# chenjianqu/dynamic_vins

Measured on AMD Instinct MI355X. Metric: stereo frames/sec (track+BA), higher is better.
Workload: dtype f64; 1 GPU; synthetic 1280x720 stereo @20 Hz + IMU @200 Hz, ZED intrinsics with distortion, figure-8 in a textured box room, max_cnt 250, min_dist 25, flow_back 1, 10 solver iterations, BA + marginalization on every frame; mode=raw, config=zed, parallelism=replicas x1 (independent sequences, no collective), landmarks_in_window=266, features_per_frame=250, warmup_requested=5, gpu_max_hw_queues=4, frames=resident in HBM before the timed region

## Files before the change

### dynamic_vins_amd/csrc/be_api.hip

```cpp
#include <algorithm>
#include <atomic>
#include <condition_variable>
#include <mutex>
#include "dv_ctx.h"
#include "be_kernels.h"

static_assert(sizeof(dv_ba_factor) == sizeof(BeFactor), "public/private factor layouts must match");
static_assert(sizeof(dv_ba_lm) == sizeof(BeLm), "public/private landmark layouts must match");
static_assert(sizeof(dv_ba_prior) == sizeof(BePriorHdr), "public/private prior layouts must match");

static int be_ensure(dv_ctx* ctx, int nfac) {
    BeWork& w = ctx->be;
    if (w.ready && nfac <= w.fac_cap) return 0;
    const int fac_cap = std::max(nfac, BE_MAX_LM * BE_MAX_OBS_FACTORS);
    size_t off = 0;
    auto take = [&](size_t bytes) { size_t o = off; off += (bytes + 255) / 256 * 256; return o; };
    const size_t n = BE_MAX_STATE;
    size_t o_ctl = take(sizeof(BeCtl)), o_x = take(sizeof(BeState)), o_imu = take(sizeof(BeImu) * BE_WIN), o_pr = take(sizeof(BePriorHdr)), o_i = take(4 * 4 * n),
           o_mt = take(4 * BE_MARG_TAB_INTS), o_lm = take(sizeof(BeLm) * BE_MAX_LM), o_fac = take(sizeof(BeFactor) * (size_t)fac_cap);
    const size_t upload_bytes = off;
    size_t o_c = take(sizeof(BeState)),
           o_pA = take(8 * (size_t)BE_MAX_PRIOR * BE_MAX_PRIOR), o_pb = take(8 * BE_MAX_PRIOR),
           o_pA2 = take(8 * (size_t)BE_MAX_PRIOR * BE_MAX_PRIOR), o_pb2 = take(8 * BE_MAX_PRIOR), o_ms = take(64), o_c0 = take(64),
           o_pk = take(8 * (size_t)BE_PK_SIZE * BE_PK_STRIDE), o_io = take(8 * (size_t)BE_WIN * IMU_OUT_STRIDE), o_po = take(8 * (BE_MAX_PRIOR + 1)),
           o_cc = take(8 * (BE_MAX_LM + BE_WIN + 1)), o_ob = take(4 * BE_MAX_LM), o_hd = take(8 * n * n), o_sc = take(8 * n * n), o_g = take(8 * 2 * n),
           o_pk1 = take(8 * (size_t)BE_PK_SIZE * BE_PK_STRIDE), o_io1 = take(8 * (size_t)BE_WIN * IMU_OUT_STRIDE), o_po1 = take(8 * (BE_MAX_PRIOR + 1)),
           o_hd1 = take(8 * n * n), o_sc1 = take(8 * n * n), o_g1 = take(8 * 2 * n),
           o_v = take(8 * 4 * n), o_vl = take(8 * 4 * (size_t)BE_MAX_LM);
    DV_CHECK(w.block.ensure(off));
    uint8_t* b = (uint8_t*)w.block.p;
    w.ctl = (BeCtl*)(b + o_ctl); w.x = (BeState*)(b + o_x); w.cand = (BeState*)(b + o_c); w.fac = (BeFactor*)(b + o_fac); w.lm = (BeLm*)(b + o_lm);
    w.imu = (BeImu*)(b + o_imu); w.prior = (BePriorHdr*)(b + o_pr);
    w.priorA_buf[0] = (double*)(b + o_pA); w.priorb_buf[0] = (double*)(b + o_pb); w.priorA_buf[1] = (double*)(b + o_pA2); w.priorb_buf[1] = (double*)(b + o_pb2);
    w.prior_cur = 0; w.priorA = w.priorA_buf[0]; w.priorb = w.priorb_buf[0]; w.prior_resident = false;
    w.marg_tab = (int32_t*)(b + o_mt); w.marg_scal = (double*)(b + o_ms); w.prior_c0 = (double*)(b + o_c0);
    w.packets[0] = (double*)(b + o_pk); w.imu_out[0] = (double*)(b + o_io); w.prior_out[0] = (double*)(b + o_po); w.cand_cost = (double*)(b + o_cc); w.lm_obs = (int32_t*)(b + o_ob);
    w.Hd[0] = (double*)(b + o_hd); w.Sc[0] = (double*)(b + o_sc); w.gvec[0] = (double*)(b + o_g);
    w.packets[1] = (double*)(b + o_pk1); w.imu_out[1] = (double*)(b + o_io1); w.prior_out[1] = (double*)(b + o_po1);
    w.Hd[1] = (double*)(b + o_hd1); w.Sc[1] = (double*)(b + o_sc1); w.gvec[1] = (double*)(b + o_g1);
    double* v = (double*)(b + o_v); w.scale_p = v; w.diag_p = v + n; w.grad_p = v + 2 * n; w.gn_p = v + 3 * n;
    double* vl = (double*)(b + o_vl); w.scale_l = vl; w.diag_l = vl + BE_MAX_LM; w.grad_l = vl + 2 * BE_MAX_LM; w.gn_l = vl + 3 * BE_MAX_LM;
    int32_t* iv = (int32_t*)(b + o_i); w.prior_col = iv; w.col_kind = iv + n; w.col_frame = iv + 2 * n; w.col_comp = iv + 3 * n;
    w.fac_cap = fac_cap;
    w.up_ctl = o_ctl; w.up_x = o_x; w.up_imu = o_imu; w.up_prior = o_pr; w.up_idx = o_i; w.up_mt = o_mt; w.up_lm = o_lm; w.up_fac = o_fac;
    const size_t need = upload_bytes + sizeof(BeState) + sizeof(BeCtl) + 4096;
    if (w.pinned_bytes < need) {
        if (w.pinned) (void)hipHostFree(w.pinned);
        w.pinned = nullptr;
        DV_CHECK(hipHostMalloc(&w.pinned, need, hipHostMallocDefault));
        w.pinned_bytes = need;
    }
    w.dl_off = upload_bytes;
    if (!w.ev_state) DV_CHECK(hipEventCreateWithFlags(&w.ev_state, hipEventDisableTiming));
    if (const char* e = std::getenv("DVINS_GPU_REJECT")) w.gpu_reject = std::atoi(e) != 0;
// ... 449 lines not shown
    if (ctx->dist.transport != 0) {
        const DvDist& dd = ctx->dist;
        sh.on = 1; sh.rank = dd.rank; sh.world = dd.world;
        sh.cap = std::max(1, (P->nlm + dd.world - 1) / dd.world);
        sh.lo = std::min(P->nlm, dd.rank * sh.cap); sh.hi = std::min(P->nlm, sh.lo + sh.cap);
        sh.len = BE_XS_LEN;
        sh.xsend = (double*)dd.xsend.p; sh.xrecv = (const double*)dd.xrecv.p;
        sh.qf[0] = (double*)dd.qf.p; sh.qf[1] = sh.qf[0] + BE_QF_LEN;
        ea.lm_lo = sh.lo; ea.lm_hi = sh.hi;
    }
    for (int k = 0; k < 2; ++k) { ea.packets[k] = w.packets[k]; ea.imu_out[k] = w.imu_out[k]; ea.prior_out[k] = w.prior_out[k]; }
    BeSolveArgs sa{};
    sa.ctl = w.ctl; sa.x = w.x; sa.cand = w.cand; sa.lm = w.lm; sa.imu = w.imu; sa.prior = w.prior; sa.priorA = w.priorA; sa.dims = d;
    sa.cand_cost = w.cand_cost; sa.lm_obs = w.lm_obs;
    for (int k = 0; k < 2; ++k) { sa.packets[k] = w.packets[k]; sa.imu_out[k] = w.imu_out[k]; sa.prior_out[k] = w.prior_out[k]; sa.Hd[k] = w.Hd[k]; sa.Sc[k] = w.Sc[k]; sa.gvec[k] = w.gvec[k]; }
    sa.scale_p = w.scale_p; sa.diag_p = w.diag_p; sa.grad_p = w.grad_p; sa.gn_p = w.gn_p; sa.scale_l = w.scale_l; sa.diag_l = w.diag_l; sa.grad_l = w.grad_l; sa.gn_l = w.gn_l;
    sa.prior_col = w.prior_col; sa.col_kind = w.col_kind; sa.col_frame = w.col_frame; sa.col_comp = w.col_comp;
    sa.xnorm2_extra = P->x_norm2_extra; sa.sh = sh; sa.xt = xt;
    sa.ldl_mf16 = 0;
    if (!w.ldl_generic && !(P->free_blocks & 3)) {
        uint8_t plan[64];
        if (be_mf16_plan(d.nstate, plan)) { std::memcpy(sa.ldl_col0, plan, sizeof(plan)); sa.ldl_mf16 = 1; }
    }
    pd.rej_on = false;
    if (fused && fused->want_reject && w.gpu_reject && P->nlm > 0) {
        if (!w.rej_pinned) DV_CHECK(hipHostMalloc((void**)&w.rej_pinned, BE_MAX_LM, hipHostMallocDefault));
        BeRejectArgs& r = pd.rej;
        r.st = w.cand; r.fac = w.fac; r.lm = w.lm; r.nlm = P->nlm; r.nframes = P->nframes; r.focal = fused->rej_focal; r.flags = w.rej_pinned;
        std::memcpy(r.ric, fused->rej_ric, sizeof(r.ric)); std::memcpy(r.tic, fused->rej_tic, sizeof(r.tic));
        r.ex_from_state = (P->free_blocks & 1) ? 1 : 0; r.pad = 0;
        pd.rej_on = true;
    }
    pd.xt = xt; pd.copy_ex_td = (P->free_blocks & 3) != 0;
    pd.ea = ea; pd.sa = sa; pd.fused_present = fused != nullptr; pd.fuse_accept_gauge = fused != nullptr && !ctx->batch && !sh.on ; pd.max_iters = P->max_iters; pd.g_norm = P->g_norm; pd.nframes = P->nframes; pd.use_imu = P->use_imu; pd.nlm = P->nlm;
    pd.want_raw_pose = fused && fused->want_raw_pose;
    if (fused) { std::memcpy(pd.gauge_R0, fused->R0, sizeof(pd.gauge_R0)); std::memcpy(pd.gauge_ypr0, fused->ypr0, sizeof(pd.gauge_ypr0)); std::memcpy(pd.gauge_P0, fused->P0, sizeof(pd.gauge_P0)); }
    pd.do_marg = do_marg; pd.state_bytes = state_bytes; pd.nxt = 1 - w.prior_cur;
    if (eval_only) {
        be_launch_eval(ea, BE_EVAL_X, s); be_launch_eval_ext(ea, xt, BE_EVAL_X, s);
        be_launch_reduce(sa, 0, s); be_launch_reduce_ext(sa, 0, s);
        if (sh.on) { if (be_exchange(ctx, (size_t)sh.len, s)) return -1; be_launch_shard_finalize(sa, 0, s); }
        DV_CHECK(hipGetLastError());
        return 0;
    }
    if (w.debug_hash_log && fused) {
        if (!w.dbg_pinned) DV_CHECK(hipHostMalloc((void**)&w.dbg_pinned, 64, hipHostMallocDefault));
// ... 405 lines not shown
    if (windows) *windows = B->t_windows;
    return 0;
}
int dv_batch_info(dv_batch* B, long long* batched_rounds, long long* single_rounds) {
    if (!B) return -1;
    if (batched_rounds) *batched_rounds = B->batched_rounds;
    if (single_rounds) *single_rounds = B->single_rounds;
    return 0;
}

int dv_debug_set(dv_ctx* ctx, const char* key, int value) {
    if (!ctx || !key) return -1;
    if (std::strcmp(key, "short_first_pass") == 0) { ctx->be.debug_short_first_pass = value != 0; return 0; }
    if (std::strcmp(key, "peer_timeout_ms") == 0) { ctx->dist.peer_timeout_ticks = 100000ll * std::max(value, 1); return 0; }
    if (std::strcmp(key, "batch_single_eval") == 0) { ctx->be.debug_batch_single = (ctx->be.debug_batch_single & ~1) | (value ? 1 : 0); return 0; }
    if (std::strcmp(key, "batch_single_reduce") == 0) { ctx->be.debug_batch_single = (ctx->be.debug_batch_single & ~2) | (value ? 2 : 0); return 0; }
    if (std::strcmp(key, "batch_single_tail") == 0) { ctx->be.debug_batch_single = (ctx->be.debug_batch_single & ~8) | (value ? 8 : 0); return 0; }
    if (std::strcmp(key, "batch_single_solve") == 0) { ctx->be.debug_batch_single = (ctx->be.debug_batch_single & ~4) | (value ? 4 : 0); return 0; }
    if (std::strcmp(key, "hash_light") == 0) { ctx->be.debug_hash_light = value != 0; return 0; }
    if (std::strcmp(key, "hash_log") == 0) { ctx->be.debug_hash_log = value != 0; return 0; }
    if (std::strcmp(key, "wait_tail") == 0) { ctx->be.debug_wait_tail = value != 0; return 0; }
    if (std::strcmp(key, "gpu_reject") == 0) { ctx->be.gpu_reject = value != 0; return 0; }
    if (std::strcmp(key, "c0_side") == 0) { ctx->be.c0_side = value != 0; return 0; }
    if (std::strcmp(key, "ldl_generic") == 0) { ctx->be.ldl_generic = value != 0; return 0; }
    DV_FAIL(std::string("dv_debug_set: unknown key ") + key);
}

int dv_ba_eval(dv_ctx* ctx, const dv_ba_problem* P, int* n_out, double* cost, double* S, double* g) {
    if (!ctx) return -1;
    if (!P || !n_out) DV_FAIL("dv_ba_eval: null argument");
    if (ctx->be.pend->active) DV_FAIL("dv_ba_eval: a solve is in flight");
    if (ctx->est && ctx->be.prior_resident && P->prior && P->prior->valid && P->prior_A != ctx->be.priorA_buf[ctx->be.prior_cur])
        DV_FAIL("dv_ba_eval: this ctx's estimator holds a device-resident prior; use a separate ctx for operator-level calls");
    if (be_begin_impl(ctx, const_cast<dv_ba_problem*>(P), nullptr, true)) return -1;
    BeWork& w = ctx->be;
    hipStream_t s = ctx->be_stream;
    const BePending& pd = *w.pend;
    if (pd.trivial) { w.pend->active = false; *n_out = 0; if (cost) *cost = 0; return 0; }
    const int n = pd.sa.dims.nstate, NBR = (n + 3) / 4, nblk = NBR * (NBR + 1) / 2;
    *n_out = n;
    std::vector<double> blk((size_t)nblk * 16), gv(2 * (size_t)n), lcost((size_t)std::max(P->nlm, 1)), io((size_t)std::max(P->nimu, 1) * IMU_OUT_STRIDE), pc(1);
    DV_CHECK(hipMemcpyAsync(blk.data(), w.Sc[0], 8 * blk.size(), hipMemcpyDeviceToHost, s));
    DV_CHECK(hipMemcpyAsync(gv.data(), w.gvec[0], 8 * gv.size(), hipMemcpyDeviceToHost, s));
    if (P->nlm) DV_CHECK(hipMemcpyAsync(lcost.data(), w.packets[0] + (size_t)BE_PK_COST * BE_PK_STRIDE, 8 * (size_t)P->nlm, hipMemcpyDeviceToHost, s));
    if (P->nimu) DV_CHECK(hipMemcpyAsync(io.data(), w.imu_out[0], 8 * (size_t)P->nimu * IMU_OUT_STRIDE, hipMemcpyDeviceToHost, s));
    DV_CHECK(hipMemcpyAsync(pc.data(), w.prior_out[0], 8, hipMemcpyDeviceToHost, s));
// ... 127 lines not shown
```

### dynamic_vins_amd/csrc/be_kernels.h

```cpp
#pragma once
#include <cstddef>
#include <hip/hip_runtime.h>
#include "be_factor_dev.h"

#define IMU_OUT_STRIDE 936

#define BE_XS_MSZ (66 * 36)
#define BE_XS_M(k) ((k) * BE_XS_MSZ)
#define BE_XS_V(k) (5 * BE_XS_MSZ + (k) * 66)
#define BE_XS_A (5 * BE_XS_MSZ + 8 * 66)
#define BE_XS_LEN (BE_XS_A + 16)
#define BE_XS_BUF ((BE_XS_LEN > BE_MAX_LM + 16 ? BE_XS_LEN : BE_MAX_LM + 16))
#define BE_QF_M(k) ((k) * 4356)
#define BE_QF_V(k) (4 * 4356 + (k) * 66)
#define BE_QF_A (4 * 4356 + 7 * 66)
#define BE_QF_LEN (BE_QF_A + 16)
struct BeShard { int32_t on, rank, world, lo, hi, cap, len, pad; double* xsend; const double* xrecv; double* qf[2]; };

#define BE_NX 13
#define BX_W 0
#define BX_G 13
#define BX_XX 26
#define BX_XP 195
#define BX_SIZE 1056
// ... 6 lines not shown
    BeDims dims; double g_norm;
    double* packets[2];
    double* imu_out[2];
    double* prior_out[2];
    double* cand_cost;
    int32_t* lm_obs;
    int32_t lm_lo, lm_hi;
    const double* prior_c0;
};

struct BeSolveArgs {
    BeCtl* ctl;
    BeState* x; BeState* cand;
    const BeLm* lm; const BeImu* imu; const BePriorHdr* prior; const double* priorA;
    BeDims dims;
    const double* packets[2]; const double* imu_out[2]; const double* prior_out[2]; const double* cand_cost; const int32_t* lm_obs;
    double* Hd[2];
    double* Sc[2];
    double* gvec[2];
    double* scale_p; double* diag_p; double* grad_p; double* gn_p;
    double* scale_l; double* diag_l; double* grad_l; double* gn_l;
    int32_t* prior_col;
    int32_t* col_kind; int32_t* col_frame; int32_t* col_comp;
    uint8_t ldl_col0[64]; int32_t ldl_mf16, ldl_pad;
    BeShard sh;
    double xnorm2_extra;
    BeExt xt;
};

struct BeMargArgs {
    const BeState* x; int nframes, nlm, nimu;
    const BeFactor* fac; const BeLm* lm; const BeImu* imu;
    const BePriorHdr* prior; const double* priorA; const double* priorb;
    const int32_t* prior_map;
    const int32_t* imu_map;
    const int32_t* dim_slot;
    const int32_t* dim_comp;
    int D, m; double g_norm;
    double* outA; double* outb; double* out_scalars;
    double* W; double* part; double* psum;
    int pose_dim[BE_NF], ex_dim[2], td_dim;
    int c0_mode;
    double* sum; double* lm_h; int anchor;
    double* imu_w;
    double* c0_out;
    const int32_t* lm_sel;
    uint8_t mf_plan[64]; int32_t mf16, mf_n;
};

struct BeGaugeArgs {
// ... 7 lines not shown
#if defined(__HIPCC__)
#include "wave_dpp.h"
using namespace be;
__device__ inline void be_frame_geom_dev(const BeState* s, int nframes, FrameGeom* fg, m33* ric, d3* tic, int lane) {
    if (lane < nframes) { fg[lane].R = qR(Q4(s->pose[lane])); fg[lane].P = P3(s->pose[lane]); }
    if (lane >= 32 && lane < 34) { ric[lane - 32] = qR(Q4(s->ex[lane - 32])); tic[lane - 32] = P3(s->ex[lane - 32]); }
}

__device__ inline void be_prior_dx_dev(const BePriorHdr* p, const BeState* s, double* dx, int lane, int nthreads) {
    for (int b = lane; b < p->nblocks; b += nthreads) {
        const BePriorBlock pb = p->blocks[b];
        const double* x0 = p->x0[b];
        if (pb.type == 0 || pb.type == 2) {
            const double* x = pb.type == 0 ? s->pose[pb.idx] : s->ex[pb.idx];
            for (int k = 0; k < 3; ++k) dx[pb.off + k] = x[k] - x0[k];
            const quat dq = qmul(qinv(Q4(x0)), Q4(x));
            d3 v = qvec(dq) * 2.0;
            if (!(dq.w >= 0)) v = -v;
            dx[pb.off + 3] = v.x; dx[pb.off + 4] = v.y; dx[pb.off + 5] = v.z;
        } else if (pb.type == 1) {
            for (int k = 0; k < 9; ++k) dx[pb.off + k] = s->sb[pb.idx][k] - x0[k];
        } else dx[pb.off] = s->td - x0[0];
    }
}

__device__ __forceinline__ void be_accept_body(const BeSolveArgs& a) {
    BeCtl* ctl = a.ctl;
    const BeCtl c = *ctl;
    __shared__ double red[4];
    __shared__ int s_accept;
    const int tid = threadIdx.x;
    __syncthreads();
    if (c.done || !c.pending) return;
    if (tid == 0) { ctl->slots = c.slots + 1; ctl->pending = 0; s_accept = 0; }
    const int iter = c.iter + 1;
    const int ncost = a.dims.nlm + a.dims.nimu + 1;
    double part = 0;
    {
        double cv[4];
#pragma unroll
        for (int u = 0; u < 4; ++u) cv[u] = a.cand_cost[tid + 256 * u < ncost ? tid + 256 * u : 0];
#pragma unroll
        for (int u = 0; u < 4; ++u) if (tid + 256 * u < ncost) part += cv[u];
    }
    part = wave_sum_f64(part);
    if ((tid & 63) == 0) red[tid >> 6] = part;
// ... 81 lines not shown
```

### dynamic_vins_amd/csrc/be_solve.hip

```cpp
#include <hip/hip_runtime.h>
#include <cfloat>
#include <algorithm>
#include <cstring>
#include <cstdlib>
#include "be_kernels.h"
#include "dev_once.h"
#include "wave_dpp.h"
#include "be_mf16.h"

using namespace be;

#ifdef BE_RED_TS
__device__ long long be_red_ts[64];
#define RTS(k) do { if (threadIdx.x == 0) be_red_ts[k] = wall_clock64(); } while (0)
extern "C" int dv_debug_red_ts(long long* out) { return hipMemcpyFromSymbol(out, HIP_SYMBOL(be_red_ts), sizeof(long long) * 64) == hipSuccess ? 0 : -1; }
#else
#define RTS(k) do {} while (0)
#endif
#define RED_THREADS 448
#define RED_PAIRS (BE_NF * (BE_NF + 1) / 2)
__device__ const unsigned char RED_PAIR_TAB[RED_PAIRS] = {
    150, 152, 51, 132, 98, 166, 170, 112, 147, 85, 68, 65, 32, 168, 49, 167, 118, 153, 66, 129, 96, 130, 165, 144, 33, 148, 67, 48, 102, 162, 161, 0, 97,
    133, 50, 16, 101, 134, 17, 119, 99, 84, 114, 64, 80, 100, 163, 160, 145, 149, 115, 131, 82, 164, 81, 151, 113, 117, 116, 128, 34, 136, 83, 169, 146, 135 };
__device__ __forceinline__ void red_pair(int bx, int& fi, int& fj) { const int t = RED_PAIR_TAB[bx]; fi = t >> 4; fj = t & 15; }
// ... 271 lines not shown
            if (threadIdx.x < 11 || threadIdx.x == 12) for (int w = 0; w < RED_THREADS / 64; ++w) v += s_red[w][threadIdx.x];
            else if (threadIdx.x == 11) for (int w = 0; w < RED_THREADS / 64; ++w) v = fmax(v, s_red[w][11]);
            a.sh.xsend[BE_XS_A + threadIdx.x] = v;
        }
        return;
    }
    if (eb == 0 && c.first && !SHARD)
        for (int l = threadIdx.x; l < nlm; l += RED_THREADS) a.scale_l[l] = 1.0 / (1.0 + sqrt(BE_PK(pk, BE_PK_H, l)));
    const int t = eb * RED_THREADS + threadIdx.x;
    if (t < n * n) {
        const int i = t / n, j = t - i * n;
        if (a.col_kind[i] == 0 && a.col_kind[j] == 0) return;
        const double hd = red_dense_h(a, rc, imu_out, i, j);
        Hd[t] = hd;
        if ((j >> 2) <= (i >> 2)) Sc[blk_pos(i, j, (n + 3) >> 2)] = hd;
    } else if (t < n * n + n) {
        const int i = t - n * n;
        if (a.col_kind[i] == 0) return;
        gvec[i] = red_dense_g(a, rc, imu_out, prior_out, i); gvec[n + i] = 0.0;
    }
    if (bx == RED_PAIRS + 3) RTS(9);
}

__global__ __launch_bounds__(RED_THREADS) void be_reduce_kernel(BeSolveArgs a, int spec) { be_reduce_body<false>(a, spec, blockIdx.x); }
__global__ __launch_bounds__(RED_THREADS) void be_reduce_shard_kernel(BeSolveArgs a, int spec) { be_reduce_body<true>(a, spec, blockIdx.x); }
__global__ __launch_bounds__(RED_THREADS) void be_reduce_batch_kernel(const BeSolveArgs* __restrict__ tab, int spec) {
    const DV_CONSTANT BeSolveArgs& a = *reinterpret_cast<const DV_CONSTANT BeSolveArgs*>(reinterpret_cast<uintptr_t>(tab + blockIdx.y));
    const int n = a.dims.nstate;
    if ((int)blockIdx.x >= RED_PAIRS + (n * n + n + RED_THREADS - 1) / RED_THREADS) return;
    be_reduce_body<false>(a, spec, blockIdx.x);
}
__global__ __launch_bounds__(RED_THREADS) __attribute__((amdgpu_waves_per_eu(6, 8))) void be_reduce_batch_occ_kernel(const BeSolveArgs* __restrict__ tab, int spec) {
    const DV_CONSTANT BeSolveArgs& a = *reinterpret_cast<const DV_CONSTANT BeSolveArgs*>(reinterpret_cast<uintptr_t>(tab + blockIdx.y));
    const int n = a.dims.nstate;
    if ((int)blockIdx.x >= RED_PAIRS + (n * n + n + RED_THREADS - 1) / RED_THREADS) return;
    be_reduce_body<false>(a, spec, blockIdx.x);
}
void be_launch_reduce_batch(const BeSolveArgs* tab_dev, int n_win, int max_n, int spec, hipStream_t s) {
    static const int occ_env = [] { const char* e = std::getenv("DVINS_REDUCE_OCC"); return e ? (e[0] != '0' ? 1 : 0) : -1; }();
    const bool occ = occ_env < 0 ? n_win >= 12 : occ_env != 0;
    const dim3 grid((RED_PAIRS + (max_n * max_n + max_n + RED_THREADS - 1) / RED_THREADS + 7) & ~7, n_win);
    if (occ) hipLaunchKernelGGL(be_reduce_batch_occ_kernel, grid, dim3(RED_THREADS), 0, s, tab_dev, spec);
    else hipLaunchKernelGGL(be_reduce_batch_kernel, grid, dim3(RED_THREADS), 0, s, tab_dev, spec);
}
void be_launch_reduce(const BeSolveArgs& a, int spec, hipStream_t s) {
    const int n = a.dims.nstate;
    const int total = n * n + n;
    if (a.sh.on) hipLaunchKernelGGL(be_reduce_shard_kernel, dim3(RED_PAIRS + (total + RED_THREADS - 1) / RED_THREADS + 1), dim3(RED_THREADS), 0, s, a, spec);
    else hipLaunchKernelGGL(be_reduce_kernel, dim3(RED_PAIRS + (total + RED_THREADS - 1) / RED_THREADS), dim3(RED_THREADS), 0, s, a, spec);
}

#define FIN_THREADS 256
__global__ __launch_bounds__(FIN_THREADS) void be_shard_finalize_kernel(BeSolveArgs a, int spec) {
    const BeCtl c = *a.ctl;
    if (c.done) return;
    int set = c.cur;
    if (spec && c.pending) set ^= 1;
    else if (!c.need_eval && !c.chol_fail) return;
    const int n = a.dims.nstate, W = a.sh.world, len = a.sh.len, t = threadIdx.x;
    const double* xr = a.sh.xrecv;
    double* qf = a.sh.qf[set];
    auto rsum = [&](int e) { double v = 0.0; for (int r = 0; r < W; ++r) v += xr[(size_t)r * len + e]; return v; };
    if (blockIdx.x < RED_PAIRS) {
        int fi, fj; red_pair(blockIdx.x, fi, fj);
        const bool in_win = fi < a.dims.nframes && fj < a.dims.nframes;
        const int ci0 = in_win ? a.dims.pose_col[fi] : -1, cj0 = in_win ? a.dims.pose_col[fj] : -1;
        const bool valid = ci0 >= 0 && cj0 >= 0;
        if (t < 36) {
            const int ci = t / 6, q = t - ci * 6, e = blockIdx.x * 36 + t, i66 = fi * 6 + ci, j66 = fj * 6 + q;
            const double v0 = valid ? rsum(BE_XS_M(0) + e) : 0.0, v2 = valid ? rsum(BE_XS_M(2) + e) : 0.0, v3 = valid ? rsum(BE_XS_M(3) + e) : 0.0, v4 = valid ? rsum(BE_XS_M(4) + e) : 0.0;
            qf[BE_QF_M(0) + i66 * 66 + j66] = v0; qf[BE_QF_M(1) + i66 * 66 + j66] = v2; qf[BE_QF_M(2) + i66 * 66 + j66] = v3; qf[BE_QF_M(3) + i66 * 66 + j66] = v4;
            if (fi != fj) { qf[BE_QF_M(0) + j66 * 66 + i66] = v0; qf[BE_QF_M(1) + j66 * 66 + i66] = v2; qf[BE_QF_M(2) + j66 * 66 + i66] = v3; qf[BE_QF_M(3) + j66 * 66 + i66] = v4; }
// ... 570 lines not shown
        if (k - R >= kend) bs_ld<SEG, R>(Lm, k - R, lane, cb);
        __builtin_amdgcn_sched_barrier(0);
        bs_ap<SEG, R>(ca, k, lane, x0, x1, x2);
        __builtin_amdgcn_sched_barrier(0);
        if (k - R >= kend) {
            if (k - 2 * R >= kend) bs_ld<SEG, R>(Lm, k - 2 * R, lane, ca);
            __builtin_amdgcn_sched_barrier(0);
            bs_ap<SEG, R>(cb, k - R, lane, x0, x1, x2);
            __builtin_amdgcn_sched_barrier(0);
        }
    }
    return 64 * SEG - 1;
}
template <int ROWS>
__device__ __forceinline__ void bs_rows(const double* Lm, int kt, int lane, double& x0, double& x1, double& x2) {
    const int seg = kt >> 6;
    if (seg == 0) bs_chunk<0, ROWS>(Lm, kt, lane, x0, x1, x2);
    else if (seg == 1) bs_chunk<1, ROWS>(Lm, kt, lane, x0, x1, x2);
    else bs_chunk<2, ROWS>(Lm, kt, lane, x0, x1, x2);
}

template <int NSLOT, bool MF16>
__global__ __launch_bounds__(SOL_THREADS) void be_solve_kernel(BeSolveArgs a, int spec) {
    constexpr bool SHARD = false;
#include "be_solve_body.inc"
}
template <int NSLOT, bool MF16>
__global__ __launch_bounds__(SOL_THREADS) void be_solve_batch_kernel(const BeSolveArgs* __restrict__ tab, int spec) {
    const BeSolveArgs& a = tab[blockIdx.x];
    constexpr bool SHARD = false;
#include "be_solve_body.inc"
}
__global__ __launch_bounds__(SOL_THREADS) void be_solve_shard_kernel(BeSolveArgs a, int spec) {
    constexpr int NSLOT = 1; constexpr bool MF16 = true, SHARD = true;
#include "be_solve_body.inc"
}

static size_t solve_smem(int n) {
    const size_t tri = (size_t)n * (n + 1) / 2;
    return (tri + 9 * (size_t)n + 72 + 80 + 8 + 1536) * sizeof(double);
}
static size_t solve_smem_mf16(int n) {
    const size_t NB = ((size_t)n + 16) >> 4, nt = NB * (NB + 1) / 2;
    return (std::max<size_t>(nt * 256, 3072) + 9 * (size_t)n + 72 + 80 + 8 + 1024 + 3 * 16 * NB) * sizeof(double);
}
bool be_mf16_plan(int n, uint8_t* plan , bool check_solve_lds) {
    const int NB = (n + 16) >> 4, W = SOL_THREADS / 64;
    if (NB > MF_MAXNB || (check_solve_lds && solve_smem_mf16(n) > 160 * 1024 - 512)) return false;
    int load[SOL_THREADS / 64] = { 0 };
    std::memset(plan, 0xFF, (size_t)W * 4);
    for (int j = 1; j < NB; ++j) plan[j * 4 + load[j]++] = (uint8_t)((j << 4) | (j - 1));
    for (int J = 0; J < NB - 1; ++J) {
        int el[SOL_THREADS / 64], ne = 0;
        for (int w = 0; w < W; ++w) if ((w == 0 || w >= NB || J < w) && w != J + 1 && load[w] < 4) el[ne++] = w;
        auto key = [&](int w) { return ((1 <= w && w < NB) ? w - 1 : NB) * 1024 + load[w] * 32 + w; };
        std::sort(el, el + ne, [&](int x, int y) { return key(x) < key(y); });
        if (ne < NB - 2 - J) return false;
// ... 44 lines not shown
```

### dynamic_vins_amd/csrc/be_solve_body.inc

```
    extern __shared__ __attribute__((aligned(16))) double sm[];
    BeCtl* ctl = a.ctl;
    BeCtl c = *ctl;
    const int n = a.dims.nstate, nlm = a.dims.nlm, tid = threadIdx.x;
    const int lm0 = SHARD ? a.sh.lo : 0, nown = SHARD ? a.sh.hi - a.sh.lo : nlm;
    if (c.done) return;
    __shared__ int s_pcol[BE_NF], s_scol[BE_NF];
    if (tid < BE_NF) { s_pcol[tid] = tid < a.dims.nframes ? a.dims.pose_col[tid] : -1; s_scol[tid] = tid < a.dims.nframes ? a.dims.sb_col[tid] : -1; }
    __shared__ int s_xcol[MF16 ? 1 : 16]; __shared__ double qx[MF16 ? 1 : 16];
    bool xt_on = false;
    if constexpr (!MF16) { xt_on = a.xt.on != 0; if (tid >= 64 && tid < 80) s_xcol[tid - 64] = (xt_on && tid - 64 < BE_NX) ? a.xt.xcol[tid - 64] : -1; }
    TS(15);
    const int cur_spec = (spec && c.pending) ? (c.cur ^ 1) : c.cur;
    double dec_cv[4] = { 0.0, 0.0, 0.0, 0.0 };
    if (MF16 && spec && c.pending && tid < 256) {
        const int ncost0 = nlm + a.dims.nimu + 1;
#pragma unroll
        for (int u = 0; u < 4; ++u) dec_cv[u] = a.cand_cost[tid + 256 * u < ncost0 ? tid + 256 * u : 0];
    }
    mf_d4 mfU[MF_SLOTS];
    double pre_h = 0.0, pre_g0 = 0.0, pre_g1 = 0.0, pre_s = 0.0;
    if (MF16 && !(c.reuse && !(spec && c.pending))) {
        mf_prefetch(a.Sc[cur_spec], reinterpret_cast<const uint8_t*>(a.ldl_col0), n, mfU);
        if (tid < n) { pre_h = a.Hd[cur_spec][(size_t)tid * n + tid]; pre_g0 = a.gvec[cur_spec][tid]; pre_g1 = a.gvec[cur_spec][n + tid]; pre_s = a.scale_p[tid]; }
    }
    if (spec && c.pending) {
        __shared__ double red4[4];
        const int ncost = nlm + a.dims.nimu + 1;
        double part = 0;
        if (tid < 256) {
            double cv[4];
#pragma unroll
            for (int u = 0; u < 4; ++u) cv[u] = MF16 ? dec_cv[u] : a.cand_cost[tid + 256 * u < ncost ? tid + 256 * u : 0];
#pragma unroll
            for (int u = 0; u < 4; ++u) if (tid + 256 * u < ncost) part += cv[u];
        }
        part = wave_sum_f64(part);
        if (tid < 256 && (tid & 63) == 0) red4[tid >> 6] = part;
        lds_barrier();
        const double cand_cost = red4[0] + red4[1] + red4[2] + red4[3];
        c.slots += 1; c.iter += 1; c.cand_cost = cand_cost; c.invalid = 0; c.pending = 0;
        bool done = false, accept = false; int term = 0;
        if (c.step_norm <= 1e-8 * (c.x_norm + 1e-8)) { done = true; term = 1; }
        else if (fabs(c.x_cost - cand_cost) <= 1e-6 * c.x_cost) { done = true; term = 1; }
        else {
            const double rel = (c.x_cost - cand_cost) / c.model_cost_change;
            if (rel > 1e-3) {
                accept = true;
                double radius = c.radius;
                if (rel < 0.25) radius *= 0.5;
                if (rel > 0.75) radius = fmax(radius, 3.0 * c.dogleg_norm);
                c.radius = radius; c.mu = fmax(1e-8, 2.0 * c.mu / 10.0);
                c.x_cost = cand_cost; c.successful += 1; c.reuse = 0; c.need_eval = 0; c.cur ^= 1;
            } else {
                c.radius = c.radius * 0.5; c.reuse = 1; c.need_eval = 0;
                if (c.radius < 1e-32) { done = true; term = 1; }
            }
            if (!done && c.iter >= c.max_iters) { done = true; term = 0; }
        }
        if (accept) {
            double* dst = reinterpret_cast<double*>(a.x);
            const double* src = reinterpret_cast<const double*>(a.cand);
            const int used = (int)(offsetof(BeState, inv_depth) / sizeof(double)) + nlm;
            for (int k = tid; k < used; k += SOL_THREADS) dst[k] = src[k];
        }
        if (done) { c.done = 1; c.termination = term; }
        if (tid == 0) *ctl = c;
        if (done) return;
        lds_barrier();
    }
    const int mf_nb = (n + 16) >> 4;
    const int npk = MF16 ? (mf_nb * (mf_nb + 1) / 2 * 256 > 3072 ? mf_nb * (mf_nb + 1) / 2 * 256 : 3072) : n * (n + 1) / 2;
    double* Lm = sm;
    double* v_s = Lm + npk;
    double* v_d = v_s + n;
    double* v_grad = v_d + n;
    double* v_gn = v_grad + n;
    double* v_t = v_gn + n;
    double* v_t2 = v_t + n;
    double* v_x = v_t2 + n;
    double* zfin = v_x + n;
    double* dvec = zfin + n;
    double* q66 = dvec + n;
    double* red = q66 + 72;
    double* misc = red + 80;
    double* scratch = MF16 ? Lm : misc + 8;
    MfLds mf; mf.Tl = Lm; mf.gat = misc + 8; mf.dv = mf.gat + 1024; mf.iv = mf.dv + 16 * mf_nb; mf.yv = mf.iv + 16 * mf_nb;
    double* PL = scratch, *PD = scratch + 4 * 184;
    double* dinfo = red;
    __shared__ int s_fail;
    const double mu = c.mu;
// ... 73 lines not shown
        if (warm_up) {
        double warm = 0.0;
        const int lpr = (nlm + 15) >> 4;
        for (int e = t; e < 66 * lpr; e += nt) { const int q = e / lpr, l16 = e - q * lpr; warm += __builtin_nontemporal_load(&BE_PK(pk, BE_PK_W + q, l16 * 16)); }
        for (int e = t; e < (n * n + 15) >> 4; e += nt) warm += __builtin_nontemporal_load(Hd + (size_t)e * 16);
        const int nst = ((int)(offsetof(BeState, inv_depth) / sizeof(double)) + nlm + 15) >> 4;
        for (int e = t; e < nst; e += nt) warm += __builtin_nontemporal_load(reinterpret_cast<const double*>(a.x) + (size_t)e * 16);
        if (warm == 1.2345e-300) misc[6] = warm;
        }
    };
    if (!c.reuse) {
        for (int i = tid; i < n; i += SOL_THREADS) {
            const bool pre = MF16 && cur_spec == c.cur;
            const double hii = pre ? pre_h : Hd[(size_t)i * n + i];
            const double s = c.first ? 1.0 / (1.0 + sqrt(hii)) : (pre ? pre_s : a.scale_p[i]);
            double d2 = hii * s * s; d2 = fmin(fmax(d2, 1e-6), 1e32);
            const double d = sqrt(d2);
            const double g0 = pre ? pre_g0 : gvec[i];
            v_s[i] = s; v_d[i] = d; v_grad[i] = g0 * s / d;
            v_x[i] = g0 - (pre ? pre_g1 : gvec[n + i]);
            if (!MF16) { if (c.first) a.scale_p[i] = s; a.diag_p[i] = d; a.grad_p[i] = v_grad[i]; }
        }
        lds_barrier();
        auto cost_and_tolerance = [&]() -> bool {
            if (c.first) {
                double part = 0;
                if (!SHARD) for (int l = tid; l < nlm; l += SOL_THREADS) part += BE_PK(pk, BE_PK_COST, l);
                for (int k = tid; k < a.dims.nimu; k += SOL_THREADS) part += imu_out[(size_t)k * IMU_OUT_STRIDE];
                if (tid == 0) part += prior_out[0];
                if (SHARD && tid == 0) part += qfc[BE_QF_A + 10];
                const double xc = block_sum(part, red);
                if (tid == 0) { ctl->x_cost = xc; ctl->initial_cost = xc; }
            }
            {
                double gm = 0;
                for (int i = tid; i < n; i += SOL_THREADS) gm = fmax(gm, fabs(gvec[i]));
                if (!SHARD) for (int l = tid; l < nlm; l += SOL_THREADS) gm = fmax(gm, fabs(BE_PK(pk, BE_PK_G, l)));
                else if (tid == 0) gm = fmax(gm, qfc[BE_QF_A + 11]);
    #pragma unroll
                for (int o = 32; o > 0; o >>= 1) gm = fmax(gm, __shfl_xor(gm, o));
                __syncthreads();
                if ((tid & 63) == 0) red[tid >> 6] = gm;
                __syncthreads();
                gm = 0; for (int k = 0; k < SOL_THREADS / 64; ++k) gm = fmax(gm, red[k]);
                __syncthreads();
                if (gm <= 1e-10) { if (tid == 0) { ctl->done = 1; ctl->termination = 1; ctl->first = 0; } return true; }
// ... 48 lines not shown
            for (int k = 0; k < SOL_THREADS / 64; ++k) { gm = fmax(gm, red[k]); xc += red[16 + k]; }
            if (c.first && tid == 0) { ctl->x_cost = xc; ctl->initial_cost = xc; }
            if (gm <= 1e-10) { if (tid == 0) { ctl->done = 1; ctl->termination = 1; ctl->first = 0; } return; }
        }
        TS(24);
        if (MF16) for (int i = tid; i < n; i += SOL_THREADS) { if (c.first) a.scale_p[i] = v_s[i]; a.diag_p[i] = v_d[i]; a.grad_p[i] = v_grad[i]; }
        TS(7);
        for (int i = tid; i < n; i += SOL_THREADS) { v_gn[i] = -v_d[i] * v_x[i]; a.gn_p[i] = v_gn[i]; v_t[i] = v_s[i] * v_x[i]; }
        lds_barrier();
        gather66(v_t);
        wdot_all();
        if (lm_live) {
            const double rho = 1.0 / (lm_h + mu * lm_diag * lm_diag / (lm_scale * lm_scale));
            lm_wgn = wd[tid];
            const double yl = rho / lm_scale * (lm_g - lm_wgn);
            lm_gn = -lm_diag * yl;
            a.gn_l[lmi] = lm_gn;
        }
        lds_barrier();
    } else {
        for (int i = tid; i < n; i += SOL_THREADS) { v_s[i] = a.scale_p[i]; v_d[i] = a.diag_p[i]; v_grad[i] = a.grad_p[i]; v_gn[i] = a.gn_p[i]; }
        if (lm_live) { lm_h = BE_PK(pk, BE_PK_H, lmi); lm_g = BE_PK(pk, BE_PK_G, lmi); lm_scale = a.scale_l[lmi]; lm_diag = a.diag_l[lmi]; lm_grad = a.grad_l[lmi]; lm_gn = a.gn_l[lmi]; }
        __syncthreads();
    }
    TS(8);
    double p_gg = 0, p_nn = 0, p_gn = 0;
    for (int i = tid; i < n; i += SOL_THREADS) { p_gg += v_grad[i] * v_grad[i]; p_nn += v_gn[i] * v_gn[i]; p_gn += v_grad[i] * v_gn[i]; }
    if (!SHARD && lm_live) { p_gg += lm_grad * lm_grad; p_nn += lm_gn * lm_gn; p_gn += lm_grad * lm_gn; }
    double f_Q2 = 0, f_Q6 = 0, f_Q9 = 0, f_L2 = 0, f_LGS = 0, f_L5 = 0, f_L6 = 0, f_L8 = 0, f_L9 = 0;
    __shared__ double vq[SHARD ? 72 : 1];
    if (SHARD) {
        if (tid < 66) { const int fa = tid / 6, r = tid - fa * 6; const int col = s_pcol[fa]; vq[tid] = col >= 0 ? -(v_s[col + r] / v_d[col + r]) * v_gn[col + r] : 0.0; }
        lds_barrier();
        double q2 = 0, q6 = 0, q9 = 0;
        for (int e = tid; e < 4356; e += SOL_THREADS) { const int i = e / 66, j = e - i * 66; const double vv = vq[i] * vq[j]; q2 += qfc[BE_QF_M(1) + e] * vv; q6 += qfc[BE_QF_M(2) + e] * vv; q9 += qfc[BE_QF_M(3) + e] * vv; }
        double l5[5] = { q2, q6, q9, 0, 0 }, l4[4] = { 0, 0, 0, 0 };
        if (tid < 66) { const double v = vq[tid]; l5[3] = v * qfc[BE_QF_V(1) + tid]; l5[4] = v * qfc[BE_QF_V(0) + tid]; l4[0] = v * qfc[BE_QF_V(3) + tid]; l4[1] = v * qfc[BE_QF_V(4) + tid]; l4[2] = v * qfc[BE_QF_V(5) + tid]; l4[3] = v * qfc[BE_QF_V(6) + tid]; }
        block_sum_n_dpp<5>(l5, red);
        block_sum_n_dpp<4>(l4, red);
        f_Q2 = l5[0]; f_Q6 = l5[1]; f_Q9 = l5[2]; f_L2 = l5[3]; f_LGS = l5[4]; f_L5 = l4[0]; f_L6 = l4[1]; f_L8 = l4[2]; f_L9 = l4[3];
        if (tid == 0) {
            const double* A = qfc + BE_QF_A;
            p_gg += A[0]; p_nn += (A[1] - 2.0 * f_L2) + f_Q2; p_gn += f_LGS - A[2];
        }
    }
    double sv3[3] = {p_gg, p_nn, p_gn};
// ... 189 lines not shown
```

### dynamic_vins_amd/csrc/dv_ctx.h

```cpp
#pragma once
#include "dv_internal.h"
#include "be_types.h"
#include "be_kernels.h"
#include <cmath>
#include <cstring>
#include <chrono>
#include <deque>
#include <map>
#include <memory>
#include <mutex>
#include <string>
#include <vector>

struct DevBuf {
    void* p = nullptr; size_t bytes = 0;
    hipError_t ensure(size_t n) {
        if (n <= bytes) return hipSuccess;
        if (p) (void)hipFree(p);
        p = nullptr; bytes = 0;
        hipError_t e = hipMalloc(&p, n);
        if (e == hipSuccess) bytes = n;
        return e;
    }
    void release() { if (p) (void)hipFree(p); p = nullptr; bytes = 0; }
// ... 42 lines not shown
struct MargPlan {
    int mode = -1, D = 0, m = 0, n = 0, nimu = 0, nsel = 0;
    bool empty = false;
    int pose_dim[BE_NF], sb_dim[BE_NF], ex_dim[2], td_dim;
    int32_t tab[BE_MARG_TAB_INTS];
};

struct BePending {
    bool want_raw_pose = false;
    bool deferred = false; int first_slots = 0;
    bool rej_on = false; BeRejectArgs rej{};
    hipEvent_t ev_state_ext = nullptr;
    bool fuse_accept_gauge = false;
    bool active = false, trivial = false, do_marg = false, fused_present = false, marg_in_flight = false, marg_check_due = false; int scal_slot = 0, check_slot = 0; size_t state_bytes = 0; int nxt = 0; MargPlan pl;
    BeExt xt{}; bool copy_ex_td = false;
    BeEvalArgs ea; BeSolveArgs sa; int max_iters = 0, nframes = 0, use_imu = 0, nlm = 0; double g_norm = 0, gauge_R0[9], gauge_ypr0[3], gauge_P0[3];
    std::chrono::steady_clock::time_point t_begin, t_up, t_enq;
};

struct BeWork {
    std::unique_ptr<BePending> pend = std::make_unique<BePending>();
    bool ready = false;
    DevBuf block;
    BeCtl* ctl = nullptr; BeState* x = nullptr; BeState* cand = nullptr;
    BeFactor* fac = nullptr; BeLm* lm = nullptr; BeImu* imu = nullptr; BePriorHdr* prior = nullptr; double* priorA = nullptr; double* priorb = nullptr;
    double* packets[2] = { nullptr, nullptr }; double* imu_out[2] = { nullptr, nullptr }; double* prior_out[2] = { nullptr, nullptr }; double* cand_cost = nullptr; int32_t* lm_obs = nullptr;
    double* Hd[2] = { nullptr, nullptr }; double* Sc[2] = { nullptr, nullptr }; double* gvec[2] = { nullptr, nullptr };
    double* scale_p = nullptr; double* diag_p = nullptr; double* grad_p = nullptr; double* gn_p = nullptr;
    double* scale_l = nullptr; double* diag_l = nullptr; double* grad_l = nullptr; double* gn_l = nullptr;
    int32_t* prior_col = nullptr; int32_t* col_kind = nullptr; int32_t* col_frame = nullptr; int32_t* col_comp = nullptr;
    int fac_cap = 0;
    DevBuf marg_buf;
    DevBuf xpk_buf;
    void* pinned = nullptr; size_t pinned_bytes = 0;
    size_t up_ctl = 0, up_x = 0, up_imu = 0, up_prior = 0, up_idx = 0, up_mt = 0, up_lm = 0, up_fac = 0, dl_off = 0;
    double* priorA_buf[2] = { nullptr, nullptr }; double* priorb_buf[2] = { nullptr, nullptr }; int prior_cur = 0;
    bool prior_resident = false;
    hipEvent_t ev_state = nullptr;
    hipStream_t c0_stream = nullptr; hipEvent_t ev_margA = nullptr, ev_c0 = nullptr; bool c0_side = false, c0_pending = false;
    double* prior_c0 = nullptr;
    int marg_form = 0;
    DevBuf eig_spec; bool eig_ran = false;
    int32_t* marg_tab = nullptr; double* marg_scal = nullptr;
    long long marg_checked = 0; double marg_last[4] = { 0, 0, 0, 0 };
    long long marg_clamped = 0;
    bool debug_short_first_pass = false, ldl_generic = false, debug_wait_tail = false; int debug_batch_single = 0; bool debug_hash_log = false, debug_hash_light = false;
    std::vector<unsigned long long> dbg_dev_log; unsigned long long* dbg_pinned = nullptr; unsigned long long dbg_solve_no = 0;
    static constexpr int DBG_RANGES = 16, DBG_SLOTS = 16;
    unsigned long long* dbg_slots = nullptr; std::vector<unsigned long long> dbg_slot_log;
    bool gpu_reject = true; uint8_t* rej_pinned = nullptr;
    std::vector<const double*> sqrt_hint;
};

bool be_imu_sqrt_info(const double* cov15x15, double* U15x15);

struct BeFused {
    int marg_mode = -1;
    double R0[9], ypr0[3], P0[3];
    dv_ba_prior new_prior;
    double diag[4] = { 0, 0, 0, 0 };
    bool want_raw_pose = false;
    bool want_reject = false; double rej_ric[2][9], rej_tic[2][3], rej_focal = 0; const uint8_t* rej_flags = nullptr;
    double raw_pose[77];
};
int be_solve_fused(dv_ctx* ctx, dv_ba_problem* P, dv_ba_summary* summary, BeFused* fused);
void be_batch_detach(dv_ctx* ctx);
struct DvFrontBatch;
DvFrontBatch*& be_batch_front(struct dv_batch* B);
int be_batch_index(struct dv_batch* B);
// ... 106 lines not shown
```

Measured before the change: 1206 frames/s.

## Move speculative accept/reject decision into an extra reduce-kernel block

Adds one extra block to the reduce kernel. In the speculative single-context MF16 path it sums the candidate costs, runs the trust-region accept/reject decision, copies the accepted candidate state into x, and writes the resulting control record to a separate ctl_dec buffer. The solve kernel then adopts that precomputed control record instead of doing the cost reduction, decision and state copy at its start. It writes the record back to ctl after its first barriers, which moves serial work off the solve kernel's critical path. This adds an extra buffer and a second control copy, with some risk of ordering subtlety between the reduce block's writes to x and other blocks.

```diff
diff --git a/dynamic_vins_amd/csrc/be_api.hip b/dynamic_vins_amd/csrc/be_api.hip
--- a/dynamic_vins_amd/csrc/be_api.hip
+++ b/dynamic_vins_amd/csrc/be_api.hip
@@ -26,10 +26,10 @@
            o_cc = take(8 * (BE_MAX_LM + BE_WIN + 1)), o_ob = take(4 * BE_MAX_LM), o_hd = take(8 * n * n), o_sc = take(8 * n * n), o_g = take(8 * 2 * n),
            o_pk1 = take(8 * (size_t)BE_PK_SIZE * BE_PK_STRIDE), o_io1 = take(8 * (size_t)BE_WIN * IMU_OUT_STRIDE), o_po1 = take(8 * (BE_MAX_PRIOR + 1)),
            o_hd1 = take(8 * n * n), o_sc1 = take(8 * n * n), o_g1 = take(8 * 2 * n),
-           o_v = take(8 * 4 * n), o_vl = take(8 * 4 * (size_t)BE_MAX_LM);
+           o_v = take(8 * 4 * n), o_vl = take(8 * 4 * (size_t)BE_MAX_LM), o_cd = take(sizeof(BeCtl));
     DV_CHECK(w.block.ensure(off));
     uint8_t* b = (uint8_t*)w.block.p;
-    w.ctl = (BeCtl*)(b + o_ctl); w.x = (BeState*)(b + o_x); w.cand = (BeState*)(b + o_c); w.fac = (BeFactor*)(b + o_fac); w.lm = (BeLm*)(b + o_lm);
+    w.ctl = (BeCtl*)(b + o_ctl); w.ctl_dec = (BeCtl*)(b + o_cd); w.x = (BeState*)(b + o_x); w.cand = (BeState*)(b + o_c); w.fac = (BeFactor*)(b + o_fac); w.lm = (BeLm*)(b + o_lm);
     w.imu = (BeImu*)(b + o_imu); w.prior = (BePriorHdr*)(b + o_pr);
     w.priorA_buf[0] = (double*)(b + o_pA); w.priorb_buf[0] = (double*)(b + o_pb); w.priorA_buf[1] = (double*)(b + o_pA2); w.priorb_buf[1] = (double*)(b + o_pb2);
     w.prior_cur = 0; w.priorA = w.priorA_buf[0]; w.priorb = w.priorb_buf[0]; w.prior_resident = false;
@@ -525,6 +525,8 @@
         uint8_t plan[64];
         if (be_mf16_plan(d.nstate, plan)) { std::memcpy(sa.ldl_col0, plan, sizeof(plan)); sa.ldl_mf16 = 1; }
     }
+    sa.ctl_dec = w.ctl_dec;
+    sa.dec_reduce = (sa.ldl_mf16 && !sh.on && !ctx->batch && !w.debug_decide_in_solve) ? 1 : 0;
     pd.rej_on = false;
     if (fused && fused->want_reject && w.gpu_reject && P->nlm > 0) {
         if (!w.rej_pinned) DV_CHECK(hipHostMalloc((void**)&w.rej_pinned, BE_MAX_LM, hipHostMallocDefault));
@@ -976,6 +978,7 @@
     if (std::strcmp(key, "wait_tail") == 0) { ctx->be.debug_wait_tail = value != 0; return 0; }
     if (std::strcmp(key, "gpu_reject") == 0) { ctx->be.gpu_reject = value != 0; return 0; }
     if (std::strcmp(key, "c0_side") == 0) { ctx->be.c0_side = value != 0; return 0; }
+    if (std::strcmp(key, "decide_in_solve") == 0) { ctx->be.debug_decide_in_solve = value != 0; return 0; }
     if (std::strcmp(key, "ldl_generic") == 0) { ctx->be.ldl_generic = value != 0; return 0; }
     DV_FAIL(std::string("dv_debug_set: unknown key ") + key);
 }
diff --git a/dynamic_vins_amd/csrc/be_kernels.h b/dynamic_vins_amd/csrc/be_kernels.h
--- a/dynamic_vins_amd/csrc/be_kernels.h
+++ b/dynamic_vins_amd/csrc/be_kernels.h
@@ -52,10 +52,11 @@
     double* scale_l; double* diag_l; double* grad_l; double* gn_l;
     int32_t* prior_col;
     int32_t* col_kind; int32_t* col_frame; int32_t* col_comp;
-    uint8_t ldl_col0[64]; int32_t ldl_mf16, ldl_pad;
+    uint8_t ldl_col0[64]; int32_t ldl_mf16, dec_reduce;
     BeShard sh;
     double xnorm2_extra;
     BeExt xt;
+    BeCtl* ctl_dec;
 };
 
 struct BeMargArgs {
@@ -109,6 +110,30 @@
             for (int k = 0; k < 9; ++k) dx[pb.off + k] = s->sb[pb.idx][k] - x0[k];
         } else dx[pb.off] = s->td - x0[0];
     }
+}
+
+__device__ __forceinline__ bool be_decide_spec(BeCtl& c, double cand_cost) {
+    c.slots += 1; c.iter += 1; c.cand_cost = cand_cost; c.invalid = 0; c.pending = 0;
+    bool done = false, accept = false; int term = 0;
+    if (c.step_norm <= 1e-8 * (c.x_norm + 1e-8)) { done = true; term = 1; }
+    else if (fabs(c.x_cost - cand_cost) <= 1e-6 * c.x_cost) { done = true; term = 1; }
+    else {
+        const double rel = (c.x_cost - cand_cost) / c.model_cost_change;
+        if (rel > 1e-3) {
+            accept = true;
+            double radius = c.radius;
+            if (rel < 0.25) radius *= 0.5;
+            if (rel > 0.75) radius = fmax(radius, 3.0 * c.dogleg_norm);
+            c.radius = radius; c.mu = fmax(1e-8, 2.0 * c.mu / 10.0);
+            c.x_cost = cand_cost; c.successful += 1; c.reuse = 0; c.need_eval = 0; c.cur ^= 1;
+        } else {
+            c.radius = c.radius * 0.5; c.reuse = 1; c.need_eval = 0;
+            if (c.radius < 1e-32) { done = true; term = 1; }
+        }
+        if (!done && c.iter >= c.max_iters) { done = true; term = 0; }
+    }
+    if (done) { c.done = 1; c.termination = term; }
+    return accept;
 }
 
 __device__ __forceinline__ void be_accept_body(const BeSolveArgs& a) {
diff --git a/dynamic_vins_amd/csrc/be_solve.hip b/dynamic_vins_amd/csrc/be_solve.hip
--- a/dynamic_vins_amd/csrc/be_solve.hip
+++ b/dynamic_vins_amd/csrc/be_solve.hip
@@ -317,7 +317,35 @@
     if (bx == RED_PAIRS + 3) RTS(9);
 }
 
-__global__ __launch_bounds__(RED_THREADS) void be_reduce_kernel(BeSolveArgs a, int spec) { be_reduce_body<false>(a, spec, blockIdx.x); }
+__device__ __forceinline__ void be_reduce_decide(const BeSolveArgs& a) {
+    BeCtl c = *a.ctl;
+    if (c.done || !c.pending) return;
+    __shared__ double red4[4];
+    const int tid = threadIdx.x, nlm = a.dims.nlm, ncost = nlm + a.dims.nimu + 1;
+    double part = 0;
+    if (tid < 256) {
+        double cv[4];
+#pragma unroll
+        for (int u = 0; u < 4; ++u) cv[u] = a.cand_cost[tid + 256 * u < ncost ? tid + 256 * u : 0];
+#pragma unroll
+        for (int u = 0; u < 4; ++u) if (tid + 256 * u < ncost) part += cv[u];
+    }
+    part = wave_sum_f64(part);
+    if (tid < 256 && (tid & 63) == 0) red4[tid >> 6] = part;
+    __syncthreads();
+    const double cand_cost = red4[0] + red4[1] + red4[2] + red4[3];
+    if (be_decide_spec(c, cand_cost)) {
+        double* dst = reinterpret_cast<double*>(a.x);
+        const double* src = reinterpret_cast<const double*>(a.cand);
+        const int used = (int)(offsetof(BeState, inv_depth) / sizeof(double)) + nlm;
+        for (int k = tid; k < used; k += RED_THREADS) dst[k] = src[k];
+    }
+    if (tid == 0) *a.ctl_dec = c;
+}
+__global__ __launch_bounds__(RED_THREADS) void be_reduce_kernel(BeSolveArgs a, int spec) {
+    if (a.dec_reduce && spec && blockIdx.x + 1 == gridDim.x) { be_reduce_decide(a); return; }
+    be_reduce_body<false>(a, spec, blockIdx.x);
+}
 __global__ __launch_bounds__(RED_THREADS) void be_reduce_shard_kernel(BeSolveArgs a, int spec) { be_reduce_body<true>(a, spec, blockIdx.x); }
 __global__ __launch_bounds__(RED_THREADS) void be_reduce_batch_kernel(const BeSolveArgs* __restrict__ tab, int spec) {
     const DV_CONSTANT BeSolveArgs& a = *reinterpret_cast<const DV_CONSTANT BeSolveArgs*>(reinterpret_cast<uintptr_t>(tab + blockIdx.y));
@@ -342,7 +370,7 @@
     const int n = a.dims.nstate;
     const int total = n * n + n;
     if (a.sh.on) hipLaunchKernelGGL(be_reduce_shard_kernel, dim3(RED_PAIRS + (total + RED_THREADS - 1) / RED_THREADS + 1), dim3(RED_THREADS), 0, s, a, spec);
-    else hipLaunchKernelGGL(be_reduce_kernel, dim3(RED_PAIRS + (total + RED_THREADS - 1) / RED_THREADS), dim3(RED_THREADS), 0, s, a, spec);
+    else hipLaunchKernelGGL(be_reduce_kernel, dim3(RED_PAIRS + (total + RED_THREADS - 1) / RED_THREADS + ((a.dec_reduce && spec) ? 1 : 0)), dim3(RED_THREADS), 0, s, a, spec);
 }
 
 #define FIN_THREADS 256
@@ -959,17 +987,17 @@
 
 template <int NSLOT, bool MF16>
 __global__ __launch_bounds__(SOL_THREADS) void be_solve_kernel(BeSolveArgs a, int spec) {
-    constexpr bool SHARD = false;
+    constexpr bool SHARD = false, DEC_RED = MF16;
 #include "be_solve_body.inc"
 }
 template <int NSLOT, bool MF16>
 __global__ __launch_bounds__(SOL_THREADS) void be_solve_batch_kernel(const BeSolveArgs* __restrict__ tab, int spec) {
     const BeSolveArgs& a = tab[blockIdx.x];
-    constexpr bool SHARD = false;
+    constexpr bool SHARD = false, DEC_RED = false;
 #include "be_solve_body.inc"
 }
 __global__ __launch_bounds__(SOL_THREADS) void be_solve_shard_kernel(BeSolveArgs a, int spec) {
-    constexpr int NSLOT = 1; constexpr bool MF16 = true, SHARD = true;
+    constexpr int NSLOT = 1; constexpr bool MF16 = true, SHARD = true, DEC_RED = false;
 #include "be_solve_body.inc"
 }
 
diff --git a/dynamic_vins_amd/csrc/be_solve_body.inc b/dynamic_vins_amd/csrc/be_solve_body.inc
--- a/dynamic_vins_amd/csrc/be_solve_body.inc
+++ b/dynamic_vins_amd/csrc/be_solve_body.inc
@@ -1,6 +1,8 @@
     extern __shared__ __attribute__((aligned(16))) double sm[];
     BeCtl* ctl = a.ctl;
     BeCtl c = *ctl;
+    const bool dec_red = DEC_RED && a.dec_reduce != 0;
+    const BeCtl cdec = *(dec_red ? a.ctl_dec : ctl);
     const int n = a.dims.nstate, nlm = a.dims.nlm, tid = threadIdx.x;
     const int lm0 = SHARD ? a.sh.lo : 0, nown = SHARD ? a.sh.hi - a.sh.lo : nlm;
     if (c.done) return;
@@ -12,7 +14,7 @@
     TS(15);
     const int cur_spec = (spec && c.pending) ? (c.cur ^ 1) : c.cur;
     double dec_cv[4] = { 0.0, 0.0, 0.0, 0.0 };
-    if (MF16 && spec && c.pending && tid < 256) {
+    if (MF16 && spec && c.pending && !dec_red && tid < 256) {
         const int ncost0 = nlm + a.dims.nimu + 1;
 #pragma unroll
         for (int u = 0; u < 4; ++u) dec_cv[u] = a.cand_cost[tid + 256 * u < ncost0 ? tid + 256 * u : 0];
@@ -23,7 +25,12 @@
         mf_prefetch(a.Sc[cur_spec], reinterpret_cast<const uint8_t*>(a.ldl_col0), n, mfU);
         if (tid < n) { pre_h = a.Hd[cur_spec][(size_t)tid * n + tid]; pre_g0 = a.gvec[cur_spec][tid]; pre_g1 = a.gvec[cur_spec][n + tid]; pre_s = a.scale_p[tid]; }
     }
-    if (spec && c.pending) {
+    bool adopt_store = false;
+    if (spec && c.pending && dec_red) {
+        c = cdec;
+        if (c.done) { if (tid == 0) *ctl = c; return; }
+        adopt_store = tid == 0;
+    } else if (spec && c.pending) {
         __shared__ double red4[4];
         const int ncost = nlm + a.dims.nimu + 1;
         double part = 0;
@@ -38,34 +45,15 @@
         if (tid < 256 && (tid & 63) == 0) red4[tid >> 6] = part;
         lds_barrier();
         const double cand_cost = red4[0] + red4[1] + red4[2] + red4[3];
-        c.slots += 1; c.iter += 1; c.cand_cost = cand_cost; c.invalid = 0; c.pending = 0;
-        bool done = false, accept = false; int term = 0;
-        if (c.step_norm <= 1e-8 * (c.x_norm + 1e-8)) { done = true; term = 1; }
-        else if (fabs(c.x_cost - cand_cost) <= 1e-6 * c.x_cost) { done = true; term = 1; }
-        else {
-            const double rel = (c.x_cost - cand_cost) / c.model_cost_change;
-            if (rel > 1e-3) {
-                accept = true;
-                double radius = c.radius;
-                if (rel < 0.25) radius *= 0.5;
-                if (rel > 0.75) radius = fmax(radius, 3.0 * c.dogleg_norm);
-                c.radius = radius; c.mu = fmax(1e-8, 2.0 * c.mu / 10.0);
-                c.x_cost = cand_cost; c.successful += 1; c.reuse = 0; c.need_eval = 0; c.cur ^= 1;
-            } else {
-                c.radius = c.radius * 0.5; c.reuse = 1; c.need_eval = 0;
-                if (c.radius < 1e-32) { done = true; term = 1; }
-            }
-            if (!done && c.iter >= c.max_iters) { done = true; term = 0; }
-        }
+        const bool accept = be_decide_spec(c, cand_cost);
         if (accept) {
             double* dst = reinterpret_cast<double*>(a.x);
             const double* src = reinterpret_cast<const double*>(a.cand);
             const int used = (int)(offsetof(BeState, inv_depth) / sizeof(double)) + nlm;
             for (int k = tid; k < used; k += SOL_THREADS) dst[k] = src[k];
         }
-        if (done) { c.done = 1; c.termination = term; }
         if (tid == 0) *ctl = c;
-        if (done) return;
+        if (c.done) return;
         lds_barrier();
     }
     const int mf_nb = (n + 16) >> 4;
@@ -185,6 +173,7 @@
             if (!MF16) { if (c.first) a.scale_p[i] = s; a.diag_p[i] = d; a.grad_p[i] = v_grad[i]; }
         }
         lds_barrier();
+        if (adopt_store) *ctl = c;
         auto cost_and_tolerance = [&]() -> bool {
             if (c.first) {
                 double part = 0;
@@ -279,6 +268,7 @@
         for (int i = tid; i < n; i += SOL_THREADS) { v_s[i] = a.scale_p[i]; v_d[i] = a.diag_p[i]; v_grad[i] = a.grad_p[i]; v_gn[i] = a.gn_p[i]; }
         if (lm_live) { lm_h = BE_PK(pk, BE_PK_H, lmi); lm_g = BE_PK(pk, BE_PK_G, lmi); lm_scale = a.scale_l[lmi]; lm_diag = a.diag_l[lmi]; lm_grad = a.grad_l[lmi]; lm_gn = a.gn_l[lmi]; }
         __syncthreads();
+        if (adopt_store) *ctl = c;
     }
     TS(8);
     double p_gg = 0, p_nn = 0, p_gn = 0;
diff --git a/dynamic_vins_amd/csrc/dv_ctx.h b/dynamic_vins_amd/csrc/dv_ctx.h
--- a/dynamic_vins_amd/csrc/dv_ctx.h
+++ b/dynamic_vins_amd/csrc/dv_ctx.h
@@ -88,7 +88,7 @@
     std::unique_ptr<BePending> pend = std::make_unique<BePending>();
     bool ready = false;
     DevBuf block;
-    BeCtl* ctl = nullptr; BeState* x = nullptr; BeState* cand = nullptr;
+    BeCtl* ctl = nullptr; BeCtl* ctl_dec = nullptr ; BeState* x = nullptr; BeState* cand = nullptr;
     BeFactor* fac = nullptr; BeLm* lm = nullptr; BeImu* imu = nullptr; BePriorHdr* prior = nullptr; double* priorA = nullptr; double* priorb = nullptr;
     double* packets[2] = { nullptr, nullptr }; double* imu_out[2] = { nullptr, nullptr }; double* prior_out[2] = { nullptr, nullptr }; double* cand_cost = nullptr; int32_t* lm_obs = nullptr;
     double* Hd[2] = { nullptr, nullptr }; double* Sc[2] = { nullptr, nullptr }; double* gvec[2] = { nullptr, nullptr };
@@ -110,7 +110,7 @@
     int32_t* marg_tab = nullptr; double* marg_scal = nullptr;
     long long marg_checked = 0; double marg_last[4] = { 0, 0, 0, 0 };
     long long marg_clamped = 0;
-    bool debug_short_first_pass = false, ldl_generic = false, debug_wait_tail = false; int debug_batch_single = 0; bool debug_hash_log = false, debug_hash_light = false;
+    bool debug_short_first_pass = false, debug_decide_in_solve = false, ldl_generic = false, debug_wait_tail = false; int debug_batch_single = 0; bool debug_hash_log = false, debug_hash_light = false;
     std::vector<unsigned long long> dbg_dev_log; unsigned long long* dbg_pinned = nullptr; unsigned long long dbg_solve_no = 0;
     static constexpr int DBG_RANGES = 16, DBG_SLOTS = 16;
     unsigned long long* dbg_slots = nullptr; std::vector<unsigned long long> dbg_slot_log;
```

Result: no change. 1203 frames/s (-0.3%).
